# danpovey/quantization

Measured on AMD Instinct MI355X. Metric: vectors encoded/sec at dim=512, 8 codebooks; uint8 codes bit-exact vs ref, higher is better.
Workload: dtype f32 (products: exact 30-bit fixed point on the i8 MFMA); 1 GPU; Quantizer.encode, dim=512, bytes_per_frame=8, codebook_size=256, refine_indexes_iters=5, batch=65536 fp32 Gaussian vectors per GPU (BASELINE.json configs[1]), seeded synthetic codebooks; global_batch=65536, parallelism=batch-sharded x1, no collective

## Files before the change

### quantization_amd/csrc/mcq_api.hip

```cpp
#include "../../include/mcq.h"
#include "../../include/mcq_residual.h"
#include "../../include/mcq_probe.h"
#include "../../include/mcq_wide.h"
#include "../../include/mcq_rerank.h"
#include "../../include/mcq_code16.h"
#include "../../include/mcq_shortlist.h"
#include "mcq_kernels.h"
#include "mcq_fix_kernels.h"
#include "mcq_loss_kernels.h"
#include "mcq_tf_kernels.h"
#include "mcq_pass16_kernels.h"
#include "mcq_train_kernels.h"
#include "mcq_search_kernels.h"
#include "mcq_range_kernels.h"
#include "mcq_wide_kernels.h"
#include "mcq_rerank_kernels.h"
#include "mcq_shortlist_kernels.h"

#include <cstdlib>
#include <iterator>
#include <type_traits>
#include <utility>
#include <vector>

// ... 304 lines not shown
    g.walk_rows = 0;
    g.out = out; g.ldo = nk;
    return launch_fgemm<FG_STORE>(g, st);
}

inline bool exact_logits_forced() {
    static const bool on = getenv("MCQ_EXACT_LOGITS") && atoi(getenv("MCQ_EXACT_LOGITS")) != 0;
    return on;
}

int launch_logits(const int8_t *xf, const int *xe, long B, const Prepared &P, int N, int K, int D, float lscale,
                  const float *lscale_ptr, float *logits, void *idx, hipStream_t st, unsigned *und_cnt = nullptr,
                  unsigned *und_list = nullptr) {
    const long nk = (long)N * K;
    FixGemm g{};
    g.A = P.Wf; g.ea = P.We; g.RA = fix_round_rows(nk); g.M = nk;
    g.B = xf; g.eb = xe; g.RB = fix_round_rows(B); g.N = B;
    g.Dq = fix_round_cols(D);
    g.walk_rows = 1;
    g.bias = P.bias; g.wmu = P.wmu; g.lscale = lscale; g.lscale_ptr = lscale_ptr;
    g.logits = logits; g.ldo = nk; g.idx = idx; g.idx_wide = K > 256 ? 1 : 0; g.K = K; g.ncb = N;
    if (und_cnt == nullptr) return launch_fgemm<FG_LOGITS>(g, st);
    if (logits != nullptr) return MCQ_EINVAL;
    g.und_cnt = und_cnt; g.und_list = und_list; g.und_cap = (unsigned)(B * N);
    const int rc = launch_fgemm<FG_SCREEN>(g, st);
    if (rc) return rc;
    FixRecheck r{};
    r.W = P.Wf; r.X = xf; r.ew = P.We; r.ex = xe; r.RW = g.RA; r.RX = g.RB; r.Dq = g.Dq;
    r.bias = P.bias; r.wmu = P.wmu; r.lscale_ptr = lscale_ptr; r.lscale = lscale;
    r.idx = idx; r.idx_wide = g.idx_wide; r.K = K; r.ncb = N; r.cnt = und_cnt; r.list = und_list; r.cap = g.und_cap;
    const long waves = B * N;
    hipLaunchKernelGGL(k_fscreen_recheck, dim3((unsigned)(waves < 4096 ? (waves + 3) / 4 : 1024)), dim3(256), 0, st, r);
    return counted_launch_rc();
}

constexpr unsigned kCapStage0 = 32768, kCapWave = 65536;
inline unsigned pass_grid(unsigned full, bool capped, unsigned cap) { return (capped && full > cap) ? cap : full; }

template <typename CT>
int launch_tf_stage0(int K, int N, const float *G, const float *XC, const CT *idx, const float *R, const float *Q, long B, int keep,
                     CT *ent, float *S, CT *fin, const int *nact, const int *map, hipStream_t st, bool capped) {
    const unsigned vgrid = (unsigned)(((B + 3) / 4) * N);
    const dim3 grid(pass_grid(vgrid, capped, kCapStage0)), block(256);
    auto with_k = [&](auto kk) {
        constexpr int KK = kk;
        return pick<1, 2, 4, 8, 16, 32, 64>(N, [&](auto nn) {
            constexpr int NN = nn;
            if constexpr ((KK == 16 && NN >= 4) || KK * NN > kMaxRows) return MCQ_EUNSUPPORTED;
            else return pick_bool(capped, [&](auto strided) {
                constexpr bool STRIDED = strided;
                hipLaunchKernelGGL((k_tf_stage0<KK, NN, STRIDED>), grid, block, 0, st, G, XC, idx, R, Q, B, keep, ent, S, fin, nact, map, vgrid);
                return counted_launch_rc();
            });
        });
    };
    if constexpr (sizeof(CT) == 1) {
        if (K == 16 && N >= 4) {
            const dim3 grid16((unsigned)((B * (N / 4) + 3) / 4));
            return pick<4, 8, 16, 32, 64>(N, [&](auto nn) {
                constexpr int NN = nn;
                hipLaunchKernelGGL((k_tf_stage0_k16<NN>), grid16, block, 0, st, G, XC, idx, R, Q, B, keep, ent, S, nact, map);
                return counted_launch_rc();
            });
        }
        return pick<16, 32, 64, 128, 256>(K, with_k);
    } else {
        return pick<512, 1024>(K, with_k);
    }
}

template <typename CT>
int launch_tf_er(int N, const float *G, const float *XC, const CT *idx, const float *xx, long B, int K, float *E, float *R,
                 float *gterms, long stride, const int *nact, const int *map, hipStream_t st, int form = -1) {
    const dim3 grid((unsigned)((B + 3) / 4)), block(256);
    const bool direct = form < 0 ? B <= 8192 : form == 0;
    return pick<1, 2, 4, 8, 16, 32, 64>(N, [&](auto nn) {
        constexpr int NN = nn, VG = 4 * (64 / NN);
        if constexpr (sizeof(CT) == 2 && NN * 512 > kMaxRows) return MCQ_EUNSUPPORTED;
        else {
            constexpr bool DENSE = sizeof(CT) == 1 && (NN == 4 || NN == 8 || NN == 16);
            if (!direct) {
                const long per = DENSE ? 256 : VG;
                hipLaunchKernelGGL((k_tf_gram_terms<NN, CT, DENSE>), dim3((unsigned)(((B + per - 1) / per) * NN)), block, 0, st, G, idx, B, K,
                                   gterms, nact, stride);
                if (const int rc = counted_launch_rc()) return rc;
                if constexpr (DENSE) {
                    hipLaunchKernelGGL((k_tf_er<NN, CT, true>), dim3((unsigned)((B + VG - 1) / VG)), block, 0, st, gterms, XC, idx, xx, B, K,
                                       E, R, nact, map, static_cast<const float *>(nullptr), stride);
                    return counted_launch_rc();
                }
            }
            hipLaunchKernelGGL((k_tf_er<NN, CT>), grid, block, 0, st, gterms, XC, idx, xx, B, K, E, R, nact, map,
                               direct ? G : static_cast<const float *>(nullptr), stride);
            return counted_launch_rc();
        }
    });
}

constexpr Pair kTfUpLists[] = {{16, 32}, {32, 32}, {32, 64}, {8, 16}, {16, 16}};
constexpr Pair kTfCombLists[] = {{16, 32}, {32, 32}, {32, 64}, {64, 64}, {8, 16}, {16, 16}};

template <typename CT>
constexpr bool tf_comb_reached(int kh, int kc, bool last) {
    const bool wide = sizeof(CT) == 2;
    if (kh == 8 || kc == 16) return !wide && !(kh == kc && last);
    if (kh == 64) return !wide;
    if (kh == kc) return !(last && wide);
    return !(kc == 64 && wide && !last);
}

int launch_tf_up(int kh, int kc, const TfLists &L, long B, int N, int u, int ntab, int per, const float *in, float *out,
                 const int *nact, hipStream_t st) {
    return pick_pair<kTfUpLists>(kh, kc, [&](auto a, auto c) {
        constexpr int KH = a, KC = c;
        hipLaunchKernelGGL((k_tf_up<KH, KC>), dim3((unsigned)(B * ntab)), dim3(64), 0, st, L, B, N, u, ntab, per, in, out, nact);
        return counted_launch_rc();
    });
}

template <typename CT>
int launch_tf_comb(int kh, int kc, const float *E, const TfLists &L, long B, int N, int v, int keep, const float *tabs,
                   CT *fin, const int *nact, hipStream_t st, bool capped) {
    if (fin == nullptr) capped = false;
    const dim3 grid(pass_grid((unsigned)(B * (N >> (v + 1))), capped, kCapWave)), block(64);
    return pick_pair<kTfCombLists>(kh, kc, [&](auto a, auto c) {
        return pick_bool(fin != nullptr, [&](auto last) {
            constexpr int KH = decltype(a)::value, KC = decltype(c)::value;
            constexpr bool LAST = last;
            if constexpr (!tf_comb_reached<CT>(KH, KC, LAST)) return MCQ_EUNSUPPORTED;
            else return pick_bool(capped, [&](auto strided) {
                constexpr bool STRIDED = strided;
                if constexpr (STRIDED && !LAST) return MCQ_EUNSUPPORTED;
                else {
                    hipLaunchKernelGGL((k_tf_comb<KH, KC, LAST, CT, STRIDED>), grid, block, 0, st, E, L, B, N, v, keep, tabs, fin, nact);
                    return counted_launch_rc();
                }
            });
        });
    });
}

enum { CAT_LOGITS = 0, CAT_XX = 1, CAT_STAGE0 = 2, CAT_XC = 3, CAT_LEVEL0 = 4, CAT_LEVEL1 = 5, CAT_TABLES = 6, CAT_COMBINE = 7,
       CAT_TABLES_UP = 8, CAT_COMBINE_UP = 9, CAT_ER = 10, CAT_LEVEL1_FUSED = 11, CAT_TAIL = 12, CAT_COUNT = 13 };
const char *const kCatNames[CAT_COUNT] = {
    "logits_product_argmax",
    "frames_to_limbs",
    "stage0_tables",
    "xc_product",
    "combine_level0",
    "combine_level1",
    "tables_level1",
    "combine_level2",
    "tables_upper_levels",
    "combine_upper_levels",
    "residual_energies",
    "level1_combines_and_tables",
    "encode_tail",
};

template <typename CT, typename F>
int pick_leaf_lists(int K, F &&f) {
    if constexpr (sizeof(CT) == 1) return pick<8, 16>(K == 16 ? 8 : 16, f);
    else return pick<16>(16, f);
}
inline bool pass16_enabled() {
    static const bool on = !(getenv("MCQ_PASS16") && atoi(getenv("MCQ_PASS16")) == 0);
    return on;
}
inline long skip_min_batch() {
    const char *v = getenv("MCQ_SKIP_MIN_BATCH");
    return v ? atol(v) : 8192;
}
constexpr long kErDenseMin = 16384;
inline long er_dense_min() {
    const char *v = getenv("MCQ_ER_DENSE_MIN");
    return v ? atol(v) : kErDenseMin;
}
constexpr long kLazyTablesMin = 16384;
inline long lazy_tables_min() {
    const char *v = getenv("MCQ_LAZY_TABLES_MIN");
    return v ? atol(v) : kLazyTablesMin;
}

template <typename CT>
int run_tf_combines(const float *G, const CT *idx_cur, CT *idx_new, const WorkspaceT<CT> &w, const TfLists &L, long B, int N,
                    int K, const int *nact, hipStream_t st, Prof *prof, bool capped) {
    const bool small = (K == 16);
    const int nlev = tf_levels(N);
    const dim3 wave(64);
    {
        const int keep = (N == 2) ? 1 : L.kc[1];
        CT *fin = (N == 2) ? idx_new : nullptr;
        const dim3 grid((unsigned)(B * (N / 2)));
        Timed t(prof, CAT_LEVEL0);
        const int rc = pick_leaf_lists<CT>(K, [&](auto kc0) {
            constexpr int KC = kc0;
            if constexpr (sizeof(CT) == 1 && KC == 16) {
                return pick_bool(capped, [&](auto strided) {
                    constexpr bool STRIDED = strided;
                    hipLaunchKernelGGL(k_tf_pair0s<STRIDED>, dim3(pass_grid(grid.x, capped, kCapWave)), wave, 0, st, G, idx_cur, w.E, L, B, N,
                                       K, keep, fin, nact);
                    return counted_launch_rc();
                });
            } else {
                hipLaunchKernelGGL((k_tf_pair0<KC, CT>), grid, wave, 0, st, G, idx_cur, w.E, L, B, N, K, keep, fin, nact);
                return counted_launch_rc();
            }
        });
        if (rc) return rc;
    }
    const bool lazy = sizeof(CT) == 1 && !small && (N == 8 || N == 16) && B >= lazy_tables_min();
    const bool fuse_l1 = (N >= 8) && !lazy;
    const bool fuse_l3 = fuse_l1 && N == 16 && small;
    if (lazy) {
        if constexpr (sizeof(CT) == 1) {
            const int ntab1 = (N >> 3) * 4, ntab3 = (N == 16) ? 16 : 1, per3 = (N == 16) ? 4 : 1;
            const unsigned pair_blocks = (unsigned)(B * (N / 4)), tab_blocks = (unsigned)(B * ntab1);
            const unsigned vgrid = tab_blocks + (N == 16 ? (unsigned)(B * ntab3) : 0u);
            const int rc = pick_bool(capped, [&](auto strided) {
                constexpr bool STRIDED = strided;
                {
                    Timed t(prof, CAT_LEVEL1);
                    hipLaunchKernelGGL((k_tf_pair1<16, 16, CT, STRIDED>), dim3(pass_grid(pair_blocks, capped, kCapWave)), wave, 0, st, G, idx_cur,
                                       w.E, L, B, N, K, L.kc[2], static_cast<CT *>(nullptr), nact);
                    if (const int rc1 = counted_launch_rc()) return rc1;
                }
                Timed t(prof, N == 16 ? CAT_TABLES_UP : CAT_TABLES);
                hipLaunchKernelGGL((k_tf_table1<16, 16, CT, true, STRIDED>), dim3(pass_grid(vgrid, capped, kCapWave)), wave, 0, st, G, idx_cur,
                                   L, B, N, K, ntab1, 2, w.tabs[0], nact, tab_blocks, ntab3, per3, w.tabs[1], vgrid);
                return counted_launch_rc();
            });
            if (rc) return rc;
        }
    } else if (fuse_l1) {
        const int keep = L.kc[2];
        const int groups2 = N >> 3, per1 = 2, ntab1 = groups2 * per1 * per1;
        const unsigned pair_blocks = (unsigned)(B * (N / 4)), tab_blocks = (unsigned)(B * ntab1);
        const int ntab3 = fuse_l3 ? 16 : 1, per3 = fuse_l3 ? 4 : 1;
        const unsigned vgrid = pair_blocks + tab_blocks + (fuse_l3 ? (unsigned)(B * ntab3) : 0u);
        const dim3 grid(pass_grid(vgrid, capped, kCapWave));
        Timed t(prof, CAT_LEVEL1_FUSED);
        const int rc = pick_leaf_lists<CT>(K, [&](auto kc0) {
            return pick_bool(capped, [&](auto strided) {
                constexpr int KC = decltype(kc0)::value;
                constexpr bool STRIDED = strided;
                hipLaunchKernelGGL((k_tf_level1<KC, KC, CT, STRIDED>), grid, wave, 0, st, G, idx_cur, w.E, L, B, N, K, keep, ntab1, per1,
                                   w.tabs[0], nact, pair_blocks, tab_blocks, ntab3, per3, w.tabs[1], vgrid);
                return counted_launch_rc();
            });
        });
        if (rc) return rc;
    } else if (N >= 4) {
        Timed t(prof, CAT_LEVEL1);
        const int rc = pick_leaf_lists<CT>(K, [&](auto kc0) {
            constexpr int KC = kc0;
            hipLaunchKernelGGL((k_tf_pair1<KC, KC, CT>), dim3((unsigned)B), wave, 0, st, G, idx_cur, w.E, L, B, N, K, 1, idx_new, nact);
            return counted_launch_rc();
        });
        if (rc) return rc;
    }
    for (int v = 2; v < nlev; ++v) {
        const int groups = N >> (v + 1);
        const bool last = (v == nlev - 1);
        const int keep = last ? 1 : L.kc[v + 1];
// ... 40 lines not shown
    float lscale;
    int N, K, D, iters;
    unsigned flags;
    hipStream_t st;
    Prof *prof;
};

struct ChunkOut {
    uint8_t *u8;
    int64_t *i64;
    uint8_t *also;
    int pack;
    uint8_t *bytes() const { return u8 ? u8 : also; }
    int bytes_pack() const { return u8 ? pack : 1; }
};

template <typename CT>
int launch_chunk_start(const EncodeCall &c, const WorkspaceT<CT> &w, const float *xc, long Bc, const int64_t *init_idx,
                       float *logits_out) {
    const int N = c.N, K = c.K, D = c.D;
    const bool screen = init_idx == nullptr && logits_out == nullptr && (c.flags & MCQ_ENCODE_EXACT_LOGITS) == 0 &&
                        !exact_logits_forced() && (size_t)Bc * N < ((size_t)1 << 31);
    unsigned *const und_cnt = reinterpret_cast<unsigned *>(w.cnt + 63), *const und_list = reinterpret_cast<unsigned *>(w.XC);
    if (init_idx == nullptr || c.iters > 0) {
        Timed t(c.prof, CAT_XX);
        const int xh = (c.flags & MCQ_ENCODE_X_FP16) ? 1 : 0;
        if (const int rc = launch_fix_rows(xc, xh, Bc, D, D, w.xf, w.xe, w.xx, c.st, c.P.mean, screen ? und_cnt : nullptr)) return rc;
    }
    if (init_idx != nullptr) {
        hipLaunchKernelGGL(k_import_indexes<CT>, dim3((unsigned)((Bc * N + 255) / 256)), dim3(256), 0, c.st, init_idx, Bc * N, K, w.idx);
        MCQ_LAUNCH_CHECK();
        if (c.prof) c.prof->untimed();
    } else {
        Timed t(c.prof, CAT_LOGITS);
        if (const int rc = launch_logits(w.xf, w.xe, Bc, c.P, N, K, D, c.lscale,
                                         (c.flags & MCQ_ENCODE_LSCALE_FROM_PREPARED) ? c.P.scales + 1 : nullptr, logits_out, w.idx, c.st,
                                         screen ? und_cnt : nullptr, und_list))
            return rc;
    }
    if (c.iters > 0) {
        Timed t(c.prof, CAT_XC);
        if (const int rc = launch_xc(w.xf, w.xe, Bc, c.P.Cf, c.P.Ce, (long)N * K, D, w.XC, c.st)) return rc;
    }
    return 0;
}

int launch_pass16(const EncodeCall &c, const WorkspaceT<uint8_t> &w, long Bc, const ChunkOut &out, uint8_t *dump = nullptr,
                  int max_wgs = 0) {
    static bool allowed16[64] = {}, allowed8[64] = {};
    int rc = allow_dynamic_lds(allowed16, reinterpret_cast<const void *>(&k_tf_pass16<16>), p16_lds_bytes<16>());
    if (rc == 0) rc = allow_dynamic_lds(allowed8, reinterpret_cast<const void *>(&k_tf_pass16<8>), p16_lds_bytes<8>());
    if (rc == 0 && dump) {
        static bool probe16[64] = {}, probe8[64] = {};
        rc = allow_dynamic_lds(probe16, reinterpret_cast<const void *>(&k_tf_pass16_probe<16>), p16_lds_bytes<16>());
        if (rc == 0) rc = allow_dynamic_lds(probe8, reinterpret_cast<const void *>(&k_tf_pass16_probe<8>), p16_lds_bytes<8>());
    }
    if (rc) return rc;
    Pass16Args a;
    a.G = c.P.G; a.XC = w.XC; a.xx = w.xx; a.Q = c.P.Q; a.idx = w.idx; a.B = Bc; a.iters = c.iters;
    a.out_i64 = out.pack == 1 ? out.i64 : nullptr;
    a.out_u8 = out.pack == 1 ? out.bytes() : nullptr;
    const long wgs = (Bc + kP16Waves - 1) / kP16Waves;
    return pick<16, 8>(c.N, [&](auto nn) {
        constexpr int NN = nn, cap = NN == 16 ? 256 : 512;
        const long lim = (max_wgs > 0 && max_wgs < cap) ? max_wgs : cap;
        const dim3 grid((unsigned)(wgs < lim ? wgs : lim)), block(64 * kP16Waves);
        if (dump) hipLaunchKernelGGL(k_tf_pass16_probe<NN>, grid, block, p16_lds_bytes<NN>(), c.st, a, dump);
        else hipLaunchKernelGGL(k_tf_pass16<NN>, grid, block, p16_lds_bytes<NN>(), c.st, a);
        return counted_launch_rc();
    });
}

template <typename CT>
struct PassState {
    CT *idx_cur, *idx_new, *idx_pk;
    int *map_cur = nullptr, *map_nxt, *map_spare, *cnt;
    const int *nact = nullptr;
    float *E_cur, *R_cur, *E_alt, *R_alt;

    PassState(const WorkspaceT<CT> &w, long Bc, bool skip)
        : idx_cur(w.idx), idx_new(skip ? w.idxB : w.idx), idx_pk(w.idxC), map_nxt(w.map[0]), map_spare(w.map[1]), cnt(w.cnt),
          E_cur(w.E), R_cur(w.R), E_alt(w.gterms), R_alt(w.gterms + ((Bc + 3) & ~3L)) {}

    void rotate(int it, bool er_ready) {
        std::swap(idx_cur, idx_pk);
        std::swap(map_cur, map_nxt);
        if (map_nxt == nullptr) map_nxt = map_spare;
        nact = cnt + it;
        if (er_ready) { std::swap(E_cur, E_alt); std::swap(R_cur, R_alt); }
    }
};

template <typename CT>
int run_one_pass(const EncodeCall &c, const WorkspaceT<CT> &w, long Bc, const PassState<CT> &s, bool last_pass, bool emit_er,
                 bool capped, bool &er_ready, const ChunkOut &out) {
    const int N = c.N, K = c.K;
    const Prepared &P = c.P;
    if (!er_ready) {
        Timed t(c.prof, CAT_ER);
        if (const int rc = launch_tf_er<CT>(N, P.G, w.XC, s.idx_cur, w.xx, Bc, K, s.E_cur, s.R_cur, w.gterms, Bc, s.nact, s.map_cur, c.st))
            return rc;
    }
    er_ready = false;
    {
        Timed t(c.prof, CAT_STAGE0);
        if (const int rc = launch_tf_stage0(K, N, P.G, w.XC, s.idx_cur, s.R_cur, P.Q, Bc, (N == 1) ? 1 : w.tf.kc[0],
                                            reinterpret_cast<CT *>(w.tf.ent), w.tf.S[0], (N == 1) ? s.idx_new : static_cast<CT *>(nullptr),
                                            s.nact, s.map_cur, c.st, capped))
            return rc;
    }
    if (N >= 2) {
        TfLists L = w.tf;
        L.map = s.map_cur;
        if (emit_er && !last_pass) {
            L.erG = P.G; L.erXC = w.XC; L.erxx = w.xx; L.erE = s.E_cur; L.erR = s.R_cur; L.erK = K;
            er_ready = true;
        }
        if (last_pass) { L.out_i64 = out.i64; L.out_u8 = out.bytes(); L.out_pack = out.bytes_pack(); }
        WorkspaceT<CT> wc = w;
        wc.E = s.E_cur; wc.R = s.R_cur;
        if (const int rc = run_tf_combines<CT>(P.G, s.idx_cur, s.idx_new, wc, L, Bc, N, K, s.nact, c.st, c.prof, capped)) return rc;
    }
    return 0;
}

template <typename CT>
int run_passes(const EncodeCall &c, const WorkspaceT<CT> &w, long Bc, bool skip, const ChunkOut &out) {
    const int N = c.N;
    PassState<CT> s(w, Bc, skip);
    if (skip) {
        hipLaunchKernelGGL(k_zero_counts, dim3(1), dim3(64), 0, c.st, w.cnt, 64);
        MCQ_LAUNCH_CHECK();
        if (c.prof) c.prof->untimed();
    }
    const bool er_in_emit = (N == 4 || N == 8 || N == 16) && !(sizeof(CT) == 1 && Bc >= er_dense_min());
    bool er_ready = false;
    for (int it = 0; it < c.iters; ++it) {
        const bool last_pass = (it + 1 == c.iters);
        const bool capped = skip && it >= 3;
        if (const int rc = run_one_pass<CT>(c, w, Bc, s, last_pass, er_in_emit, capped, er_ready, out)) return rc;
        const bool emits = N >= 2 && last_pass;
        if (skip && !emits) {
            {
                Timed t(c.prof, CAT_TAIL);
                hipLaunchKernelGGL(k_compact<CT>, dim3((unsigned)((Bc + 255) / 256)), dim3(256), 0, c.st, s.idx_cur, s.idx_new, s.map_cur,
                                   s.nact, Bc, N, last_pass ? 1 : 0, s.idx_pk, s.map_nxt, w.cnt + it, er_ready ? s.E_cur : nullptr,
                                   er_ready ? s.R_cur : nullptr, s.E_alt, s.R_alt, out.pack, out.u8, out.i64, out.also);
                MCQ_LAUNCH_CHECK();
            }
            s.rotate(it, er_ready);
        }
    }
    return 0;
}

template <typename CT>
int run_encode_t(const float *x, long B, const void *prepared, float lscale, int N, int K, int D, int iters,
                 uint8_t *out_u8, int64_t *out_i64, void *workspace, size_t workspace_bytes, hipStream_t st,
                 Prof *prof, const int64_t *init_idx, unsigned flags, float *logits_out,
                 uint8_t *codes_also ) {
    g_last_launches = 0;
    if (!domain_ok(N, K, D)) return domain_err(N, K, D);
    if (B < 0 || iters < 0 || iters > 60 || (out_u8 == nullptr) == (out_i64 == nullptr)) return MCQ_EINVAL;
    if (sizeof(CT) > 1 && (out_u8 != nullptr || codes_also != nullptr)) return MCQ_EINVAL;
    if (B == 0) return 0;
    if (!x || !prepared || !workspace) return MCQ_EINVAL;
    const size_t per = workspace_per_vector(N, K, D), slack = workspace_slack(D);
    if (workspace_bytes < slack + per) return MCQ_EWORKSPACE;
    long chunk = (long)((workspace_bytes - slack) / per);
    if (chunk > B) chunk = B;
    if (chunk < B && chunk < 128) return MCQ_EWORKSPACE;
    if (chunk < B) chunk &= ~127L;
    const EncodeCall c{prepared_view(prepared, N, K, D), lscale, N, K, D, iters, flags, st, prof};
    const int pack = (out_u8 != nullptr && K == 16 && N >= 2) ? 2 : 1;
    const bool want_skip = (flags & MCQ_ENCODE_ALL_PASSES) == 0 && iters >= 3;
    const bool use_p16 = sizeof(CT) == 1 && K == 16 && (N == 16 || N == 8) && iters > 0 && prof == nullptr && pass16_enabled();

    for (long lo = 0; lo < B; lo += chunk) {
        const long Bc = (B - lo < chunk) ? (B - lo) : chunk;
        const WorkspaceT<CT> w = carve<CT>(workspace, Bc, N, K, D);
        const ChunkOut out{out_u8 ? out_u8 + lo * (N / pack) : nullptr, out_i64 ? out_i64 + lo * N : nullptr,
                           codes_also ? codes_also + lo * N : nullptr, pack};
        const float *xc = (flags & MCQ_ENCODE_X_FP16) ? reinterpret_cast<const float *>(reinterpret_cast<const uint16_t *>(x) + lo * D)
                                                      : x + lo * D;
        if (const int rc = launch_chunk_start<CT>(c, w, xc, Bc, init_idx ? init_idx + lo * N : nullptr,
                                                  logits_out ? logits_out + lo * N * K : nullptr))
            return rc;
        bool left = false;
        if constexpr (sizeof(CT) == 1) {
            if (use_p16) {
                if (const int rc = launch_pass16(c, w, Bc, out)) return rc;
                left = out.pack == 1;
            }
        }
        if (!use_p16) {
            const bool skip = want_skip && Bc >= skip_min_batch();
            if (const int rc = run_passes<CT>(c, w, Bc, skip, out)) return rc;
            left = skip || (iters > 0 && N >= 2);
        }
        if (left) continue;
        const long outn = out.i64 ? Bc * N : Bc * (N / pack);
        Timed t(prof, CAT_TAIL);
        hipLaunchKernelGGL(k_finalize<CT>, dim3((unsigned)((outn + 255) / 256)), dim3(256), 0, st, w.idx, Bc, N, pack, out.u8, out.i64,
                           out.also);
        MCQ_LAUNCH_CHECK();
    }
    return 0;
}

int run_encode(const float *x, long B, const void *prepared, float lscale, int N, int K, int D, int iters,
               uint8_t *out_u8, int64_t *out_i64, void *workspace, size_t workspace_bytes, hipStream_t st,
               Prof *prof, const int64_t *init_idx = nullptr, unsigned flags = 0, float *logits_out = nullptr,
               uint8_t *codes_also = nullptr) {
    if (K > 256)
        return run_encode_t<uint16_t>(x, B, prepared, lscale, N, K, D, iters, out_u8, out_i64, workspace, workspace_bytes, st, prof,
                                      init_idx, flags, logits_out, codes_also);
    return run_encode_t<uint8_t>(x, B, prepared, lscale, N, K, D, iters, out_u8, out_i64, workspace, workspace_bytes, st, prof,
                                 init_idx, flags, logits_out, codes_also);
}

template <typename CT>
int test_pass(const EncodeCall &c, const float *x, long B, const int64_t *idx_in, int64_t *idx_out, const int *nact, const int *map,
              bool capped, void *workspace) {
    const WorkspaceT<CT> w = carve<CT>(workspace, B, c.N, c.K, c.D);
    if (const int rc = launch_chunk_start<CT>(c, w, x, B, idx_in, nullptr)) return rc;
    PassState<CT> s(w, B, false);
    s.nact = nact;
    s.map_cur = const_cast<int *>(map);
    bool er_ready = false;
    return run_one_pass<CT>(c, w, B, s, true, false, capped, er_ready, ChunkOut{nullptr, idx_out, nullptr, 1});
}

int db_cw_of(int D, int K) {
// ... 1648 lines not shown
```

### quantization_amd/csrc/mcq_tf_kernels.h

```cpp
#pragma once
#include "mcq_kernels.h"

#include <type_traits>

namespace mcq {

constexpr int kTfLevels = 6;

template <int K>
using tf_code_of = std::conditional_t<(K > 256), uint16_t, uint8_t>;

struct TfLists {
    uint8_t *ent;
    uint8_t *pos[kTfLevels];
    float *S[kTfLevels];
    int kc[kTfLevels];
    int64_t *out_i64;
    uint8_t *out_u8;
    int out_pack;
    const int *map;
    const float *erG, *erXC, *erxx;
    float *erE, *erR;
    int erK;
};

__device__ __forceinline__ float shfl_f(float v, int src) {
    return __int_as_float(__builtin_amdgcn_ds_bpermute(src << 2, __float_as_int(v)));
}

#ifdef MCQ_STAMPS
constexpr int kStampSlots = 8, kStampWaves = 1 << 14, kStampKernels = 4;
__device__ unsigned long long g_stamps[kStampKernels * kStampWaves * kStampSlots];
struct Stamps {
    unsigned long long t[kStampSlots];
    __device__ __forceinline__ Stamps() { for (int i = 0; i < kStampSlots; ++i) t[i] = 0; t[0] = __builtin_amdgcn_s_memtime(); }
    __device__ __forceinline__ void at(int k) { asm volatile("s_waitcnt vmcnt(0) lgkmcnt(0)" ::: "memory"); t[k] = __builtin_amdgcn_s_memtime(); }
    __device__ __forceinline__ void flush(int kernel, unsigned wg, int every) {
        if (wg % (unsigned)every != 0 || (threadIdx.x & 63) != 0 || (threadIdx.x >> 6) != 0) return;
        const unsigned slot = (wg / (unsigned)every) & (kStampWaves - 1);
        unsigned long long *d = g_stamps + ((size_t)kernel * kStampWaves + slot) * kStampSlots;
        t[kStampSlots - 1] = __builtin_amdgcn_s_memtime();
        for (int i = 0; i < kStampSlots; ++i) d[i] = t[i];
    }
};
#else
struct Stamps {
    __device__ __forceinline__ void at(int) {}
    __device__ __forceinline__ void flush(int, unsigned, int) {}
};
#endif


template <int N, typename CT>
__device__ __forceinline__ void tf_gram_terms_dense(const float *__restrict__ G, const CT *__restrict__ idx, long B, int K,
                                                    float *__restrict__ gterms, const int *__restrict__ nact, long stride);
template <int N, typename CT>
__device__ __forceinline__ void tf_er_dense(const float *__restrict__ gterms, const float *__restrict__ XC, const CT *__restrict__ idx,
                                            const float *__restrict__ xx, long B, int K, float *__restrict__ E_out,
                                            float *__restrict__ R_out, const int *__restrict__ nact, const int *__restrict__ map,
                                            long stride);

template <int N, typename CT = uint8_t, bool DENSE = false>
__global__ void __launch_bounds__(256)
k_tf_gram_terms(const float *__restrict__ G, const CT *__restrict__ idx, long B, int K, float *__restrict__ gterms,
                const int *__restrict__ nact, long stride) {
    if constexpr (DENSE) { tf_gram_terms_dense<N, CT>(G, idx, B, K, gterms, nact, stride); return; }
    constexpr int VW = 64 / N;
    if (nact) B = *nact;
    const int m = (int)(blockIdx.x % N);
    const long b = ((long)(blockIdx.x / N) * 4 + (threadIdx.x >> 6)) * VW + lane_id() / N;
    const int m2 = lane_id() % N;
    if (b >= B) return;
    const CT *id = idx + b * N;
    const int NK = N * K;
    gterms[(b * N + m) * N + m2] = G[((size_t)(m * K + id[m]) << __builtin_ctz((unsigned)NK)) + m2 * K + id[m2]];
}

template <int N, bool FROM_REG, typename CT = uint8_t>
__device__ __forceinline__ void tf_er_wave(long b, long bx, const CT *__restrict__ id, int e_reg,
                                           const float *__restrict__ gterms, const float *__restrict__ Gdirect,
                                           const float *__restrict__ XC, const float *__restrict__ xx, int K,
                                           float *__restrict__ E_out, float *__restrict__ R_out) {
    constexpr int NT = (N * N + 63) / 64;
    const int lane = lane_id();
    const int NK = N * K;
#define MCQ_ER_CODE(m) (FROM_REG ? __builtin_amdgcn_ds_bpermute((m) << 2, e_reg) : (int)id[FROM_REG ? 0 : (m)])
    float gt[NT];
#pragma unroll
    for (int j = 0; j < NT; ++j) {
        const int t = lane + 64 * j;
        const int tc = t < N * N ? t : 0;
        const float g = Gdirect ? Gdirect[(size_t)((tc / N) * K + MCQ_ER_CODE(tc / N)) * NK + (tc % N) * K + MCQ_ER_CODE(tc % N)]
                                : gterms[b * (N * N) + tc];
        gt[j] = t < N * N ? g : 0.f;
    }
    const int lm = lane < N ? lane : 0;
    const int clm = MCQ_ER_CODE(lm);
#undef MCQ_ER_CODE
    const float xt = lane < N ? XC[(size_t)bx * NK + lm * K + clm] : 0.f;
    const float xxb = xx[bx];
    float gp = gt[0];
#pragma unroll
    for (int j = 1; j < NT; ++j) gp = gp + gt[j];
    const float gsum = wave_sum_butterfly(gp), xsum = wave_sum_butterfly(xt);
    const float E = (gsum - 2.0f * xsum) + xxb;
    const int n = lane < N ? lane : 0;
    float col = 0.f, gnn = 0.f;
#pragma unroll
    for (int m = 0; m < N; ++m) {
        const float v = shfl_f(gt[(m * N) / 64], (m * N + n) & 63);
        col = (m == 0) ? v : col + v;
        if (m == n) gnn = v;
    }
    const float xo = col - xt;
    const float Rv = (E - 2.0f * xo) + gnn;
    if (lane < N) R_out[b * N + lane] = Rv;
    if (lane == 0) E_out[b] = E;
}

template <int N, typename CT = uint8_t, bool DENSE = false>
__global__ void __launch_bounds__(256)
k_tf_er(const float *__restrict__ gterms, const float *__restrict__ XC, const CT *__restrict__ idx,
        const float *__restrict__ xx, long B, int K, float *__restrict__ E_out, float *__restrict__ R_out,
        const int *__restrict__ nact, const int *__restrict__ map, const float *__restrict__ Gdirect, long stride) {
    if constexpr (DENSE) { tf_er_dense<N, CT>(gterms, XC, idx, xx, B, K, E_out, R_out, nact, map, stride); return; }
    if (nact) B = *nact;
    const long b = (long)blockIdx.x * 4 + (threadIdx.x >> 6);
    if (b >= B) return;
    const long bx = map ? (long)map[b] : b;
    tf_er_wave<N, false, CT>(b, bx, idx + b * N, 0, gterms, Gdirect, XC, xx, K, E_out, R_out);
}

constexpr int tf_gram_planes(int N) { return N / 2 + 1; }

template <int N>
__device__ __forceinline__ int tf_gram_plane(int m, int n) {
    const int d = (n - m) & (N - 1);
    const bool own = d < N / 2 || (d == N / 2 && m < N / 2);
    return own ? m * tf_gram_planes(N) + d : n * tf_gram_planes(N) + (N - d);
}

template <int NW>
__device__ __forceinline__ int tf_code_at(const uint32_t (&w)[NW], int j) {
    uint32_t x = w[0];
#pragma unroll
    for (int i = 1; i < NW; ++i) x = (j >> 2) == i ? w[i] : x;
    return (int)((x >> ((j & 3) * 8)) & 0xffu);
}

template <int N, typename CT>
__device__ __forceinline__ void tf_gram_terms_dense(const float *__restrict__ G, const CT *__restrict__ idx, long B, int K,
                                                    float *__restrict__ gterms, const int *__restrict__ nact, long stride) {
    static_assert(sizeof(CT) == 1 && (N == 4 || N == 8 || N == 16), "the dense form: 4, 8 or 16 codebooks of one-byte entries");
    constexpr int NW = N / 4, ND = tf_gram_planes(N);
    if (nact) B = *nact;
    const int m = (int)(blockIdx.x % N);
    const long b = (long)(blockIdx.x / N) * 256 + threadIdx.x;
    if (b >= B) return;
    const uint32_t *src = static_cast<const uint32_t *>(__builtin_assume_aligned(idx + b * N, N));
    uint32_t w[NW];
#pragma unroll
    for (int i = 0; i < NW; ++i) w[i] = src[i];
    const size_t NK = (size_t)N * K;
    const float *row = G + (size_t)(m * K + tf_code_at<NW>(w, m)) * NK;
    const bool half = m < N / 2;
    float g[ND];
#pragma unroll
    for (int d = 0; d < ND; ++d) {
        const int m2 = (m + d) & (N - 1);
        g[d] = (d < N / 2 || half) ? row[m2 * K + tf_code_at<NW>(w, m2)] : 0.f;
    }
#pragma unroll
    for (int d = 0; d < ND; ++d)
        if (d < N / 2 || half) gterms[(size_t)(m * ND + d) * stride + b] = g[d];
}

template <int N, typename CT>
__device__ __forceinline__ void tf_er_dense(const float *__restrict__ gterms, const float *__restrict__ XC, const CT *__restrict__ idx,
                                            const float *__restrict__ xx, long B, int K, float *__restrict__ E_out,
                                            float *__restrict__ R_out, const int *__restrict__ nact, const int *__restrict__ map,
                                            long stride) {
    static_assert(sizeof(CT) == 1 && (N == 4 || N == 8 || N == 16), "the dense form: 4, 8 or 16 codebooks of one-byte entries");
    constexpr int VW = 64 / N;
    constexpr int RS = 64 / N;
    if (nact) B = *nact;
    const int lane = lane_id(), n = lane % N;
    const long b = ((long)blockIdx.x * 4 + (threadIdx.x >> 6)) * VW + lane / N;
    if (b >= B) return;
    const long bx = map ? (long)map[b] : b;
    const float xt = XC[(size_t)bx * N * K + n * K + idx[b * N + n]];
    const float xxb = xx[bx];
    float g[N];
#pragma unroll
    for (int m = 0; m < N; ++m) g[m] = gterms[(size_t)tf_gram_plane<N>(m, n) * stride + b];
    float p[RS];
#pragma unroll
    for (int r = 0; r < RS; ++r) {
        p[r] = r < N ? g[r] : 0.f;
#pragma unroll
        for (int m = r + RS; m < N; m += RS) p[r] = p[r] + g[m];
    }
#pragma unroll
    for (int h = RS / 2; h >= 1; h >>= 1)
#pragma unroll
        for (int r = 0; r < h; ++r) p[r] = p[r] + p[r + h];
    float gsum = p[0], xsum = xt;
#pragma unroll
    for (int s = 32; s >= N; s >>= 1) xsum = xsum + 0.f;
#pragma unroll
    for (int s = N / 2; s >= 1; s >>= 1) {
        gsum = gsum + __shfl_xor(gsum, s, 64);
        xsum = xsum + __shfl_xor(xsum, s, 64);
    }
    const float E = (gsum - 2.0f * xsum) + xxb;
    float col = g[0], gnn = g[0];
#pragma unroll
    for (int m = 1; m < N; ++m) {
        col = col + g[m];
        gnn = (m == n) ? g[m] : gnn;
    }
    const float xo = col - xt;
    R_out[b * N + n] = (E - 2.0f * xo) + gnn;
    if (n == 0) E_out[b] = E;
}

template <int K, int N>
__device__ __forceinline__ void
tf_stage0_body(unsigned bid, unsigned vgrid, const float *__restrict__ G, const float *__restrict__ XC, const tf_code_of<K> *__restrict__ idx,
               const float *__restrict__ R, const float *__restrict__ Q, long B, int keep,
               tf_code_of<K> *__restrict__ ent_out, float *__restrict__ S_out, tf_code_of<K> *__restrict__ idx_final ,
               const int *__restrict__ nact, const int *__restrict__ map) {
    using CT = tf_code_of<K>;
    constexpr int CB = (int)sizeof(CT);
    constexpr int VPL = (K >= 64) ? K / 64 : 1;
    constexpr int NK = N * K;
    constexpr int CH = (N - 1 < 8) ? (N > 1 ? N - 1 : 1) : 8;
    __shared__ u64 sel[4][kSelectLdsU64];
    Stamps stp;
    if (nact) B = *nact;
    int n;
    long b;
    if constexpr (N > 8) {
        const unsigned per_phase = vgrid / (N / 8);
        const unsigned ph = bid / per_phase, r = bid - ph * per_phase;
        n = (int)(r & 7u) + 8 * (int)ph;
        b = (long)(r >> 3) * 4 + (threadIdx.x >> 6);
    } else {
        n = bid & (N - 1);
        b = (long)(bid / N) * 4 + (threadIdx.x >> 6);
    }
    if (b >= B) return;
    const int lane = lane_id();
    const bool act = VPL * lane < K;
    const int k0 = act ? VPL * lane : 0;
    const CT *id = idx + b * N;
    const float *xc = XC + ((size_t)(map ? (long)map[b] : b) * NK + n * K + k0);
    const float *q = Q + n * K + k0;
    float xcv[VPL], qv[VPL];
    if constexpr (VPL == 4) {
        const f32x4 x4 = __builtin_nontemporal_load(reinterpret_cast<const f32x4 *>(xc)), q4 = *reinterpret_cast<const f32x4 *>(q);
#pragma unroll
        for (int i = 0; i < 4; ++i) { xcv[i] = x4[i]; qv[i] = q4[i]; }
    } else if constexpr (VPL % 4 == 0) {
#pragma unroll
        for (int i4 = 0; i4 < VPL / 4; ++i4) {
            const f32x4 x4 = reinterpret_cast<const f32x4 *>(xc)[i4], q4 = reinterpret_cast<const f32x4 *>(q)[i4];
#pragma unroll
            for (int i = 0; i < 4; ++i) { xcv[4 * i4 + i] = x4[i]; qv[4 * i4 + i] = q4[i]; }
        }
    } else {
#pragma unroll
        for (int i = 0; i < VPL; ++i) { xcv[i] = xc[i]; qv[i] = q[i]; }
    }
    const float Rv = R[(long)__builtin_amdgcn_readfirstlane((int)b) * N + n];
    __builtin_amdgcn_sched_barrier(0);
    unsigned long long iw[N * CB >= 8 ? N * CB / 8 : 1];
    if constexpr (N * CB >= 8) {
        const unsigned long long *ip =
            reinterpret_cast<const unsigned long long *>(idx) + (size_t)__builtin_amdgcn_readfirstlane((int)b) * (N * CB / 8);
#pragma unroll
        for (int q8 = 0; q8 < N * CB / 8; ++q8) iw[q8] = ip[q8];
    }
    auto code = [&](int m) -> int {
        if constexpr (N * CB >= 8) return (int)((iw[(m * CB) >> 3] >> (8 * ((m * CB) & 7))) & (CB == 1 ? 0xffull : 0xffffull));
        else return (int)id[m];
    };
    float t[VPL];
#pragma unroll
    for (int i = 0; i < VPL; ++i) t[i] = 0.f;
#pragma unroll
    for (int j0 = 0; j0 < N - 1; j0 += CH) {
        float gv[CH][VPL];
#pragma unroll
        for (int u = 0; u < CH; ++u) {
            const int j = j0 + u < N - 1 ? j0 + u : N - 2;
            const int m = j < n ? j : j + 1;
            const float *p = G + ((size_t)(m * K + code(m)) * NK + n * K + k0);
            if constexpr (VPL % 4 == 0) {
#pragma unroll
                for (int i4 = 0; i4 < VPL / 4; ++i4) {
                    const f32x4 t4 = reinterpret_cast<const f32x4 *>(p)[i4];
#pragma unroll
                    for (int i = 0; i < 4; ++i) gv[u][4 * i4 + i] = t4[i];
                }
            } else {
#pragma unroll
// ... 951 lines not shown
```

Before: 14.88 million vectors/s.

## Fuse stream compaction into the dense E/R kernel and skip unchanged rows

For large one-byte batches with active-set skipping, the separate compaction kernel is replaced by a retiring E/R kernel. It compares new and old codes, writes finished codes straight to the output, and packs the changed vectors' indices, map entries and E/R into compacted slots using a ballot and an atomic counter. The gram-term kernel also skips unchanged vectors. The goal is to avoid one launch and the compaction pass over E/R, and to avoid gathering gram terms for converged vectors. In exchange it adds a block-wide atomic, extra __syncthreads, and packed-slot order that differs from the prefix-ordered compaction.

Result: no change. 14.79 million vectors/s (-0.6%).

```diff
diff --git a/quantization_amd/csrc/mcq_api.hip b/quantization_amd/csrc/mcq_api.hip
--- a/quantization_amd/csrc/mcq_api.hip
+++ b/quantization_amd/csrc/mcq_api.hip
@@ -410,18 +410,35 @@
             if (!direct) {
                 const long per = DENSE ? 256 : VG;
                 hipLaunchKernelGGL((k_tf_gram_terms<NN, CT, DENSE>), dim3((unsigned)(((B + per - 1) / per) * NN)), block, 0, st, G, idx, B, K,
-                                   gterms, nact, stride);
+                                   gterms, nact, stride, static_cast<const CT *>(nullptr));
                 if (const int rc = counted_launch_rc()) return rc;
                 if constexpr (DENSE) {
                     hipLaunchKernelGGL((k_tf_er<NN, CT, true>), dim3((unsigned)((B + VG - 1) / VG)), block, 0, st, gterms, XC, idx, xx, B, K,
-                                       E, R, nact, map, static_cast<const float *>(nullptr), stride);
+                                       E, R, nact, map, static_cast<const float *>(nullptr), stride, TfRetire{});
                     return counted_launch_rc();
                 }
             }
             hipLaunchKernelGGL((k_tf_er<NN, CT>), grid, block, 0, st, gterms, XC, idx, xx, B, K, E, R, nact, map,
-                               direct ? G : static_cast<const float *>(nullptr), stride);
+                               direct ? G : static_cast<const float *>(nullptr), stride, TfRetire{});
             return counted_launch_rc();
         }
+    });
+}
+
+int launch_tf_er_retire(int N, const float *G, const float *XC, const uint8_t *idx, const float *xx, long B, int K, float *E, float *R,
+                        float *gterms, long stride, const int *nact, const int *map, const TfRetire &rt, hipStream_t st) {
+    const dim3 block(256);
+    const bool direct = B <= 8192;
+    return pick<4, 8, 16>(N, [&](auto nn) {
+        constexpr int NN = nn, VG = 4 * (64 / NN);
+        if (!direct) {
+            hipLaunchKernelGGL((k_tf_gram_terms<NN, uint8_t, true, true>), dim3((unsigned)(((B + 255) / 256) * NN)), block, 0, st, G, idx, B, K,
+                               gterms, nact, stride, rt.idx_old);
+            if (const int rc = counted_launch_rc()) return rc;
+        }
+        hipLaunchKernelGGL((k_tf_er<NN, uint8_t, true, true>), dim3((unsigned)((B + VG - 1) / VG)), block, 0, st, gterms, XC, idx, xx, B, K,
+                           E, R, nact, map, direct ? G : static_cast<const float *>(nullptr), stride, rt);
+        return counted_launch_rc();
     });
 }
 
@@ -508,6 +525,11 @@
 inline long lazy_tables_min() {
     const char *v = getenv("MCQ_LAZY_TABLES_MIN");
     return v ? atol(v) : kLazyTablesMin;
+}
+constexpr long kErCompactMin = 16384;
+inline long er_compact_min() {
+    const char *v = getenv("MCQ_ER_COMPACT_MIN");
+    return v ? atol(v) : kErCompactMin;
 }
 
 template <typename CT>
@@ -714,12 +736,12 @@
         : idx_cur(w.idx), idx_new(skip ? w.idxB : w.idx), idx_pk(w.idxC), map_nxt(w.map[0]), map_spare(w.map[1]), cnt(w.cnt),
           E_cur(w.E), R_cur(w.R), E_alt(w.gterms), R_alt(w.gterms + ((Bc + 3) & ~3L)) {}
 
-    void rotate(int it, bool er_ready) {
+    void rotate(int it, bool er_ready, bool er_moved) {
         std::swap(idx_cur, idx_pk);
         std::swap(map_cur, map_nxt);
         if (map_nxt == nullptr) map_nxt = map_spare;
         nact = cnt + it;
-        if (er_ready) { std::swap(E_cur, E_alt); std::swap(R_cur, R_alt); }
+        if (er_ready && er_moved) { std::swap(E_cur, E_alt); std::swap(R_cur, R_alt); }
     }
 };
 
@@ -766,13 +788,25 @@
         if (c.prof) c.prof->untimed();
     }
     const bool er_in_emit = (N == 4 || N == 8 || N == 16) && !(sizeof(CT) == 1 && Bc >= er_dense_min());
+    const bool er_retires = skip && sizeof(CT) == 1 && (N == 4 || N == 8 || N == 16) && !er_in_emit && out.pack == 1 &&
+                            Bc >= er_compact_min();
     bool er_ready = false;
     for (int it = 0; it < c.iters; ++it) {
         const bool last_pass = (it + 1 == c.iters);
         const bool capped = skip && it >= 3;
         if (const int rc = run_one_pass<CT>(c, w, Bc, s, last_pass, er_in_emit, capped, er_ready, out)) return rc;
         const bool emits = N >= 2 && last_pass;
-        if (skip && !emits) {
+        if (skip && !emits && er_retires) {
+            if constexpr (sizeof(CT) == 1) {
+                Timed t(c.prof, CAT_ER);
+                const TfRetire rt{s.idx_cur, s.idx_pk, s.map_nxt, w.cnt + it, out.u8, out.i64, out.also};
+                if (const int rc = launch_tf_er_retire(N, c.P.G, w.XC, s.idx_new, w.xx, Bc, c.K, s.E_cur, s.R_cur, w.gterms, Bc, s.nact,
+                                                       s.map_cur, rt, c.st))
+                    return rc;
+            }
+            er_ready = true;
+            s.rotate(it, er_ready, false);
+        } else if (skip && !emits) {
             {
                 Timed t(c.prof, CAT_TAIL);
                 hipLaunchKernelGGL(k_compact<CT>, dim3((unsigned)((Bc + 255) / 256)), dim3(256), 0, c.st, s.idx_cur, s.idx_new, s.map_cur,
@@ -780,7 +814,7 @@
                                    er_ready ? s.R_cur : nullptr, s.E_alt, s.R_alt, out.pack, out.u8, out.i64, out.also);
                 MCQ_LAUNCH_CHECK();
             }
-            s.rotate(it, er_ready);
+            s.rotate(it, er_ready, true);
         }
     }
     return 0;
diff --git a/quantization_amd/csrc/mcq_tf_kernels.h b/quantization_amd/csrc/mcq_tf_kernels.h
--- a/quantization_amd/csrc/mcq_tf_kernels.h
+++ b/quantization_amd/csrc/mcq_tf_kernels.h
@@ -51,20 +51,37 @@
 #endif
 
 
-template <int N, typename CT>
+struct TfRetire {
+    const uint8_t *idx_old;
+    uint8_t *idx_packed;
+    int *map_next;
+    int *cnt_next;
+    uint8_t *out_u8;
+    int64_t *out_i64;
+    uint8_t *codes_also;
+};
+
+template <int N, typename CT, bool RETIRE>
 __device__ __forceinline__ void tf_gram_terms_dense(const float *__restrict__ G, const CT *__restrict__ idx, long B, int K,
-                                                    float *__restrict__ gterms, const int *__restrict__ nact, long stride);
+                                                    float *__restrict__ gterms, const int *__restrict__ nact, long stride,
+                                                    const CT *__restrict__ idx_old);
 template <int N, typename CT>
 __device__ __forceinline__ void tf_er_dense(const float *__restrict__ gterms, const float *__restrict__ XC, const CT *__restrict__ idx,
                                             const float *__restrict__ xx, long B, int K, float *__restrict__ E_out,
                                             float *__restrict__ R_out, const int *__restrict__ nact, const int *__restrict__ map,
                                             long stride);
-
-template <int N, typename CT = uint8_t, bool DENSE = false>
+template <int N>
+__device__ __forceinline__ void tf_er_retire(const float *__restrict__ gterms, const float *__restrict__ XC, const uint8_t *__restrict__ idx,
+                                             const float *__restrict__ xx, long B, int K, float *__restrict__ E_out,
+                                             float *__restrict__ R_out, const int *__restrict__ nact, const int *__restrict__ map,
+                                             const float *__restrict__ Gdirect, long stride, const TfRetire &rt);
+
+template <int N, typename CT = uint8_t, bool DENSE = false, bool RETIRE = false>
 __global__ void __launch_bounds__(256)
 k_tf_gram_terms(const float *__restrict__ G, const CT *__restrict__ idx, long B, int K, float *__restrict__ gterms,
-                const int *__restrict__ nact, long stride) {
-    if constexpr (DENSE) { tf_gram_terms_dense<N, CT>(G, idx, B, K, gterms, nact, stride); return; }
+                const int *__restrict__ nact, long stride, const CT *__restrict__ idx_old) {
+    static_assert(DENSE || !RETIRE, "the retiring flavour is a dense one");
+    if constexpr (DENSE) { tf_gram_terms_dense<N, CT, RETIRE>(G, idx, B, K, gterms, nact, stride, idx_old); return; }
     constexpr int VW = 64 / N;
     if (nact) B = *nact;
     const int m = (int)(blockIdx.x % N);
@@ -118,11 +135,13 @@
     if (lane == 0) E_out[b] = E;
 }
 
-template <int N, typename CT = uint8_t, bool DENSE = false>
+template <int N, typename CT = uint8_t, bool DENSE = false, bool RETIRE = false>
 __global__ void __launch_bounds__(256)
 k_tf_er(const float *__restrict__ gterms, const float *__restrict__ XC, const CT *__restrict__ idx,
         const float *__restrict__ xx, long B, int K, float *__restrict__ E_out, float *__restrict__ R_out,
-        const int *__restrict__ nact, const int *__restrict__ map, const float *__restrict__ Gdirect, long stride) {
+        const int *__restrict__ nact, const int *__restrict__ map, const float *__restrict__ Gdirect, long stride, const TfRetire rt) {
+    static_assert(DENSE || !RETIRE, "the retiring flavour is a dense one");
+    if constexpr (RETIRE) { tf_er_retire<N>(gterms, XC, idx, xx, B, K, E_out, R_out, nact, map, Gdirect, stride, rt); return; }
     if constexpr (DENSE) { tf_er_dense<N, CT>(gterms, XC, idx, xx, B, K, E_out, R_out, nact, map, stride); return; }
     if (nact) B = *nact;
     const long b = (long)blockIdx.x * 4 + (threadIdx.x >> 6);
@@ -148,9 +167,10 @@
     return (int)((x >> ((j & 3) * 8)) & 0xffu);
 }
 
-template <int N, typename CT>
+template <int N, typename CT, bool RETIRE>
 __device__ __forceinline__ void tf_gram_terms_dense(const float *__restrict__ G, const CT *__restrict__ idx, long B, int K,
-                                                    float *__restrict__ gterms, const int *__restrict__ nact, long stride) {
+                                                    float *__restrict__ gterms, const int *__restrict__ nact, long stride,
+                                                    const CT *__restrict__ idx_old) {
     static_assert(sizeof(CT) == 1 && (N == 4 || N == 8 || N == 16), "the dense form: 4, 8 or 16 codebooks of one-byte entries");
     constexpr int NW = N / 4, ND = tf_gram_planes(N);
     if (nact) B = *nact;
@@ -161,6 +181,13 @@
     uint32_t w[NW];
 #pragma unroll
     for (int i = 0; i < NW; ++i) w[i] = src[i];
+    if constexpr (RETIRE) {
+        const uint32_t *old = static_cast<const uint32_t *>(__builtin_assume_aligned(idx_old + b * N, N));
+        bool changed = false;
+#pragma unroll
+        for (int i = 0; i < NW; ++i) changed = changed || (old[i] != w[i]);
+        if (!changed) return;
+    }
     const size_t NK = (size_t)N * K;
     const float *row = G + (size_t)(m * K + tf_code_at<NW>(w, m)) * NK;
     const bool half = m < N / 2;
@@ -173,6 +200,40 @@
 #pragma unroll
     for (int d = 0; d < ND; ++d)
         if (d < N / 2 || half) gterms[(size_t)(m * ND + d) * stride + b] = g[d];
+}
+
+template <int N>
+__device__ __forceinline__ float tf_er_dense_sums(const float (&g)[N], float xt, float xxb, int n, float &Rv) {
+    constexpr int RS = 64 / N;
+    float p[RS];
+#pragma unroll
+    for (int r = 0; r < RS; ++r) {
+        p[r] = r < N ? g[r] : 0.f;
+#pragma unroll
+        for (int m = r + RS; m < N; m += RS) p[r] = p[r] + g[m];
+    }
+#pragma unroll
+    for (int h = RS / 2; h >= 1; h >>= 1)
+#pragma unroll
+        for (int r = 0; r < h; ++r) p[r] = p[r] + p[r + h];
+    float gsum = p[0], xsum = xt;
+#pragma unroll
+    for (int s = 32; s >= N; s >>= 1) xsum = xsum + 0.f;
+#pragma unroll
+    for (int s = N / 2; s >= 1; s >>= 1) {
+        gsum = gsum + __shfl_xor(gsum, s, 64);
+        xsum = xsum + __shfl_xor(xsum, s, 64);
+    }
+    const float E = (gsum - 2.0f * xsum) + xxb;
+    float col = g[0], gnn = g[0];
+#pragma unroll
+    for (int m = 1; m < N; ++m) {
+        col = col + g[m];
+        gnn = (m == n) ? g[m] : gnn;
+    }
+    const float xo = col - xt;
+    Rv = (E - 2.0f * xo) + gnn;
+    return E;
 }
 
 template <int N, typename CT>
@@ -182,7 +243,6 @@
                                             long stride) {
     static_assert(sizeof(CT) == 1 && (N == 4 || N == 8 || N == 16), "the dense form: 4, 8 or 16 codebooks of one-byte entries");
     constexpr int VW = 64 / N;
-    constexpr int RS = 64 / N;
     if (nact) B = *nact;
     const int lane = lane_id(), n = lane % N;
     const long b = ((long)blockIdx.x * 4 + (threadIdx.x >> 6)) * VW + lane / N;
@@ -193,35 +253,80 @@
     float g[N];
 #pragma unroll
     for (int m = 0; m < N; ++m) g[m] = gterms[(size_t)tf_gram_plane<N>(m, n) * stride + b];
-    float p[RS];
-#pragma unroll
-    for (int r = 0; r < RS; ++r) {
-        p[r] = r < N ? g[r] : 0.f;
-#pragma unroll
-        for (int m = r + RS; m < N; m += RS) p[r] = p[r] + g[m];
-    }
-#pragma unroll
-    for (int h = RS / 2; h >= 1; h >>= 1)
-#pragma unroll
-        for (int r = 0; r < h; ++r) p[r] = p[r] + p[r + h];
-    float gsum = p[0], xsum = xt;
-#pragma unroll
-    for (int s = 32; s >= N; s >>= 1) xsum = xsum + 0.f;
-#pragma unroll
-    for (int s = N / 2; s >= 1; s >>= 1) {
-        gsum = gsum + __shfl_xor(gsum, s, 64);
-        xsum = xsum + __shfl_xor(xsum, s, 64);
-    }
-    const float E = (gsum - 2.0f * xsum) + xxb;
-    float col = g[0], gnn = g[0];
-#pragma unroll
-    for (int m = 1; m < N; ++m) {
-        col = col + g[m];
-        gnn = (m == n) ? g[m] : gnn;
-    }
-    const float xo = col - xt;
-    R_out[b * N + n] = (E - 2.0f * xo) + gnn;
+    float Rv;
+    const float E = tf_er_dense_sums<N>(g, xt, xxb, n, Rv);
+    R_out[b * N + n] = Rv;
     if (n == 0) E_out[b] = E;
+}
+
+template <int N>
+__device__ __forceinline__ void tf_er_retire(const float *__restrict__ gterms, const float *__restrict__ XC, const uint8_t *__restrict__ idx,
+                                             const float *__restrict__ xx, long B, int K, float *__restrict__ E_out,
+                                             float *__restrict__ R_out, const int *__restrict__ nact, const int *__restrict__ map,
+                                             const float *__restrict__ Gdirect, long stride, const TfRetire &rt) {
+    static_assert(N == 4 || N == 8 || N == 16, "the dense form: 4, 8 or 16 codebooks of one-byte entries");
+    constexpr int VW = 64 / N, NW = N / 4;
+    __shared__ int wave_cnt[4], wg_base;
+    if (nact) B = *nact;
+    if ((long)blockIdx.x * (4 * VW) >= B) return;
+    const int lane = lane_id(), n = lane % N, wave = (int)(threadIdx.x >> 6), first = lane - n;
+    const long b = ((long)blockIdx.x * 4 + wave) * VW + lane / N;
+    const bool valid = b < B;
+    const long bs = valid ? b : 0;
+    const uint32_t *src = static_cast<const uint32_t *>(__builtin_assume_aligned(idx + bs * N, N));
+    const uint32_t *old = static_cast<const uint32_t *>(__builtin_assume_aligned(rt.idx_old + bs * N, N));
+    uint32_t w[NW];
+    bool changed = false;
+#pragma unroll
+    for (int i = 0; i < NW; ++i) {
+        w[i] = src[i];
+        changed = changed || (old[i] != w[i]);
+    }
+    changed = changed && valid;
+    const long bx = map ? (long)map[bs] : bs;
+    const int cn = tf_code_at<NW>(w, n);
+    const u64 cm = __ballot(changed && n == 0);
+    if (lane == 0) wave_cnt[wave] = __popcll(cm);
+    __syncthreads();
+    if (threadIdx.x == 0) {
+        const int total = (wave_cnt[0] + wave_cnt[1]) + (wave_cnt[2] + wave_cnt[3]);
+        wg_base = total ? atomicAdd(rt.cnt_next, total) : 0;
+    }
+    __syncthreads();
+    if (!valid) return;
+    if (!changed) {
+        if (rt.out_i64 != nullptr) {
+            rt.out_i64[bx * N + n] = cn;
+            if (rt.codes_also) rt.codes_also[bx * N + n] = (uint8_t)cn;
+        } else {
+            rt.out_u8[bx * N + n] = (uint8_t)cn;
+        }
+        return;
+    }
+    long slot = wg_base + __popcll(cm & (((u64)1 << first) - 1));
+#pragma unroll
+    for (int i = 0; i < 3; ++i) slot += i < wave ? wave_cnt[i] : 0;
+    rt.idx_packed[slot * N + n] = (uint8_t)cn;
+    if (n == 0) rt.map_next[slot] = (int)bx;
+    const size_t NK = (size_t)N * K;
+    const float xt = XC[(size_t)bx * NK + n * K + cn];
+    const float xxb = xx[bx];
+    float g[N];
+#pragma unroll
+    for (int m = 0; m < N; ++m) {
+        if (Gdirect) {
+            const int d = (n - m) & (N - 1);
+            const bool own = d < N / 2 || (d == N / 2 && m < N / 2);
+            const int r = own ? m : n, c = own ? n : m;
+            g[m] = Gdirect[(size_t)(r * K + tf_code_at<NW>(w, r)) * NK + c * K + tf_code_at<NW>(w, c)];
+        } else {
+            g[m] = gterms[(size_t)tf_gram_plane<N>(m, n) * stride + b];
+        }
+    }
+    float Rv;
+    const float E = tf_er_dense_sums<N>(g, xt, xxb, n, Rv);
+    R_out[slot * N + n] = Rv;
+    if (n == 0) E_out[slot] = E;
 }
 
 template <int K, int N>
```
